# keonlee9420/Comprehensive-Transformer-TTS

Measured on AMD Instinct MI355X. Metric: mel-frames/sec (train step) LJSpeech batch=16, 1/2/4/8 MI355X, higher is better.
Workload: dtype f32; 1 GPU; LJSpeech transformer_fs2 batch=16/GPU seq<=128->mel<=1024x80; full train step fwd+loss+bwd+clip+Adam, dropout on; workload_detail=supervised durations (BASELINE configs[1]), global_batch=16, valid_frames_per_gpu=11992, padded_frames_per_gpu=16384, launch_mode=hipgraph(fwd+bwd | clip+adam), parallelism=dp1

## Files before the change

### comprehensive-transformer-tts_amd/_lib.py

```python
import ctypes as C
import os

_HERE = os.path.dirname(os.path.abspath(__file__))
LIB_PATH = os.environ.get("CTTS_LIB") or os.path.join(_HERE, "csrc", "libctts_hip.so")

_c_f32p = C.c_void_p
_i32, _i64, _f32, _u32, _vp = C.c_int32, C.c_int64, C.c_float, C.c_uint32, C.c_void_p


class GemmDesc(C.Structure):
    _fields_ = [
        ("A", _vp), ("B", _vp), ("C", _vp),
        ("M", _i32), ("N", _i32), ("K", _i32),
        ("lda", _i64), ("ldb", _i64), ("ldc", _i64),
        ("a_kc", _i32), ("b_kc", _i32),
        ("nb0", _i32), ("nb1", _i32),
        ("sA0", _i64), ("sA1", _i64), ("sB0", _i64), ("sB1", _i64), ("sC0", _i64), ("sC1", _i64),
        ("lens", _vp),
        ("lim_m", _i32), ("lim_n", _i32), ("lim_k", _i32),
        ("conv_T", _i32), ("conv_pad", _i32), ("conv_cin", _i32), ("conv_on_b", _i32),
        ("split_k", _i32),
        ("alpha", _f32),
        ("bias", _vp),
        ("Z", _vp), ("ldz", _i64),
# ... 56 lines not shown
    ]


class PsumTask(C.Structure):
    _fields_ = [("src", _vp), ("dst", _vp), ("n", _i64), ("stride", _i64), ("count", _i32), ("alpha", _f32)]


class SplitTask(C.Structure):
    _fields_ = [("src", _vp), ("dst", _vp), ("rows", _i64), ("cols", _i64), ("ld", _i64)]


class RepackTask(C.Structure):
    _fields_ = [("src", _vp), ("dst", _vp), ("cout", _i32), ("cin", _i32), ("k", _i32)]


_SIGNATURES = {
    "ctts_conv_dgrad_weights": [C.POINTER(RepackTask), C.c_int, _vp],
    "ctts_gemm_split_plan": [C.POINTER(GemmDesc), C.POINTER(_i32), C.POINTER(_i64)],
    "ctts_gemm_route": [C.POINTER(GemmDesc), C.POINTER(GemmRouteInfo)],
    "ctts_partial_sums": [C.POINTER(PsumTask), C.c_int, _vp],
    "ctts_reduce_parts": [C.c_int, _i64, C.c_int],
    "ctts_xcd_probe": [_vp, C.c_int, _vp],
    "ctts_posembed_fwd": [_vp, _vp, _vp, _vp, _vp, _vp, _i64, C.c_int, _f32, _vp, _u32, _vp],
    "ctts_posembed_bwd": [_vp, _vp, _vp, _vp, _vp, _vp, _i64, C.c_int, _f32, _vp, _u32, C.c_int, _vp, _vp],
    "ctts_gemm": [C.POINTER(GemmDesc), _vp],
    "ctts_gemm_takes_persistent": [C.POINTER(GemmDesc)],
    "ctts_gemm_ws_enable": [C.c_int],
    "ctts_gemm_takes_weight_stationary": [C.POINTER(GemmDesc)],
    "ctts_gemm_takes_bf16_split": [C.POINTER(GemmDesc)],
    "ctts_gemm_takes_planes": [C.POINTER(GemmDesc)],
    "ctts_split_planes": [C.POINTER(SplitTask), C.c_int, _vp],
# ... 111 lines not shown
    "ctts_comm_unique_id": [_vp],
    "ctts_comm_create": [C.POINTER(_vp), _i32, _i32, _vp],
    "ctts_comm_destroy": [_vp],
    "ctts_allreduce_mean": [_vp, _i64, _vp, _vp],
}
COMM_ID_BYTES = 128
EXPORTED_SYMBOLS = sorted(list(_SIGNATURES) + ["ctts_last_error", "ctts_version", "ctts_mha_supported", "ctts_relmha_workspace_floats",
                                               "ctts_mel_spectrogram_workspace_bytes", "ctts_gemm_workspace_bytes", "ctts_workspace_bytes",
                                               "ctts_workspace_error_word", "ctts_fastformer_workspace_floats",
                                               "ctts_griffinlim_workspace_bytes", "ctts_griffinlim_state_floats",
                                               "ctts_pitch_track_workspace_bytes", "ctts_trim_silence_workspace_bytes",
                                               "ctts_dtw_workspace_bytes", "ctts_loudness_workspace_bytes", "ctts_stoi_workspace_bytes",
                                               "ctts_si_sdr_workspace_bytes", "ctts_mr_stft_workspace_bytes",
                                               "ctts_batch_tile_map_ints", "ctts_conv2d_nhwc_workspace_bytes"])
ADAM_STATE_FLOATS = 3 + 2048
ABI_VERSION = 2

_lib = None


class CttsError(RuntimeError):
    pass


def load():
    global _lib
    if _lib is not None:
        return _lib
    if not os.path.exists(LIB_PATH):
        raise CttsError(
# ... 60 lines not shown
```

### comprehensive-transformer-tts_amd/csrc/optim.hip

```cpp
#include "ctts_common.h"

namespace {

__global__ __launch_bounds__(256) void sqnorm_kernel(const float4* __restrict__ g, long n4, const float* __restrict__ gtail, int ntail,
                                                      float* __restrict__ state) {
  float acc = 0.f;
  for (long i = (long)blockIdx.x * blockDim.x + threadIdx.x; i < n4; i += (long)gridDim.x * blockDim.x) {
    const float4 v = g[i];
    acc += v.x * v.x + v.y * v.y + v.z * v.z + v.w * v.w;
  }
  if (blockIdx.x == 0 && (int)threadIdx.x < ntail) acc += gtail[threadIdx.x] * gtail[threadIdx.x];
  acc = ctts_wave_sum(acc);
  __shared__ float s[4];
  if ((threadIdx.x & 63) == 0) s[threadIdx.x >> 6] = acc;
  __syncthreads();
  if (threadIdx.x == 0) state[3 + blockIdx.x] = (s[0] + s[1]) + (s[2] + s[3]);
}

__global__ __launch_bounds__(256) void sqnorm_reduce_kernel(float* __restrict__ state, int nparts) {
  __shared__ float s[256];
  float acc = 0.f;
  for (int i = threadIdx.x; i < nparts; i += 256) acc += state[3 + i];
  s[threadIdx.x] = acc;
  __syncthreads();
// ... 1 lines not shown
    if ((int)threadIdx.x < o) s[threadIdx.x] += s[threadIdx.x + o];
    __syncthreads();
  }
  if (threadIdx.x == 0) state[0] = s[0];
}

__device__ __forceinline__ void adam_one(float& p, float g, float& m, float& v, float coef, float wd, float b1, float b2, float eps,
                                         float step_size, float inv_sqrt_bc2) {
  g = g * coef + wd * p;
  m = b1 * m + (1.f - b1) * g;
  v = b2 * v + (1.f - b2) * g * g;
  const float denom = sqrtf(v) * inv_sqrt_bc2 + eps;
  p -= step_size * (m / denom);
}

__global__ __launch_bounds__(256) void adam_kernel(float* __restrict__ p, const float* __restrict__ g, float* __restrict__ m,
                                                    float* __restrict__ v, long n, const float* __restrict__ lr, float b1, float b2,
                                                    float eps, float wd, float max_norm, const float* __restrict__ state) {
  const float total = sqrtf(state[0]);
  float coef = 1.f;
  if (max_norm > 0.f) {
    const float c = max_norm / (total + 1e-6f);
    coef = c > 1.f ? 1.f : c;
  }
  const float step = state[1] + 1.f;
  const float bc1 = 1.f - powf(b1, step), bc2 = 1.f - powf(b2, step);
  const float step_size = lr[0] / bc1, inv_sqrt_bc2 = rsqrtf(bc2);
  const long n4 = n >> 2;
  float4* p4 = reinterpret_cast<float4*>(p);
  const float4* g4 = reinterpret_cast<const float4*>(g);
  float4* m4 = reinterpret_cast<float4*>(m);
  float4* v4 = reinterpret_cast<float4*>(v);
  for (long i = (long)blockIdx.x * blockDim.x + threadIdx.x; i < n4; i += (long)gridDim.x * blockDim.x) {
    float4 pp = p4[i], mm = m4[i], vv = v4[i];
    const float4 gg = g4[i];
    adam_one(pp.x, gg.x, mm.x, vv.x, coef, wd, b1, b2, eps, step_size, inv_sqrt_bc2);
    adam_one(pp.y, gg.y, mm.y, vv.y, coef, wd, b1, b2, eps, step_size, inv_sqrt_bc2);
    adam_one(pp.z, gg.z, mm.z, vv.z, coef, wd, b1, b2, eps, step_size, inv_sqrt_bc2);
    adam_one(pp.w, gg.w, mm.w, vv.w, coef, wd, b1, b2, eps, step_size, inv_sqrt_bc2);
    p4[i] = pp; m4[i] = mm; v4[i] = vv;
  }
  if (blockIdx.x == 0) {
    const long i = (n4 << 2) + threadIdx.x;
    if (i < n) adam_one(p[i], g[i], m[i], v[i], coef, wd, b1, b2, eps, step_size, inv_sqrt_bc2);
  }
}

__global__ void adam_finalize_kernel(float* __restrict__ state) {
  state[2] = sqrtf(state[0]);
  state[1] += 1.f;
}

}

extern "C" int ctts_adam_clip_step(float* p, const float* g, float* m, float* v, int64_t n, const float* lr, float beta1, float beta2,
                                   float eps, float weight_decay, float max_norm, float* state, void* stream) {
  CTTS_REQUIRE(p && g && m && v && lr && state && n >= 0, "ctts_adam_clip_step: bad arguments");
  auto al16 = [](const void* q) { return (reinterpret_cast<uintptr_t>(q) & 15) == 0; };
  CTTS_REQUIRE(al16(p) && al16(g) && al16(m) && al16(v), "ctts_adam_clip_step: arenas must be 16-byte aligned");
  if (n == 0) return 0;
  hipStream_t st = (hipStream_t)stream;
  const long n4 = n >> 2;
  const int blocks = (int)((n4 + 255) / 256 > CTTS_ADAM_PARTIALS ? CTTS_ADAM_PARTIALS : ((n4 + 255) / 256 < 1 ? 1 : (n4 + 255) / 256));
  hipLaunchKernelGGL(sqnorm_kernel, dim3(blocks), dim3(256), 0, st, (const float4*)g, n4, g + (n4 << 2), (int)(n - (n4 << 2)), state);
  CTTS_CHECK_LAUNCH("ctts_adam_clip_step(sqnorm)");
  hipLaunchKernelGGL(sqnorm_reduce_kernel, dim3(1), dim3(256), 0, st, state, blocks);
  CTTS_CHECK_LAUNCH("ctts_adam_clip_step(sqnorm reduce)");
  hipLaunchKernelGGL(adam_kernel, dim3(blocks), dim3(256), 0, st, p, g, m, v, (long)n, lr, beta1, beta2, eps, weight_decay, max_norm, state);
  CTTS_CHECK_LAUNCH("ctts_adam_clip_step(adam)");
  hipLaunchKernelGGL(adam_finalize_kernel, dim3(1), dim3(1), 0, st, state);
  CTTS_CHECK_LAUNCH("ctts_adam_clip_step(finalize)");
  return 0;
}

namespace {
__global__ __launch_bounds__(256) void mel_l1_fwd_kernel(const float* __restrict__ p1, const float* __restrict__ p2,
                                                          const float* __restrict__ tgt, const unsigned char* __restrict__ pad,
                                                          float* __restrict__ sums, float* __restrict__ roww, long rows, int C,
                                                          unsigned char* ws, int G) {
  const int lane = threadIdx.x & 63, wave = threadIdx.x >> 6;
  float a1 = 0.f, a2 = 0.f, aw = 0.f;
  for (long r = (long)blockIdx.x * 4 + wave; r < rows; r += (long)gridDim.x * 4) {
    const bool is_pad = pad[r] != 0;
    float s_t = 0.f, s1 = 0.f, s2 = 0.f;
    for (int c = lane; c < C; c += 64) {
      const float t = is_pad ? 0.f : tgt[r * C + c];
      const float x1 = is_pad ? 0.f : p1[r * C + c], x2 = is_pad ? 0.f : p2[r * C + c];
      s_t += fabsf(t); s1 += fabsf(x1 - t); s2 += fabsf(x2 - t);
    }
// ... 54 lines not shown
```

### comprehensive-transformer-tts_amd/dp.py

```python
import torch
import torch.distributed as dist


ARENA_ALIGN = 64


def arena_offsets(params):
    offs, o = [], 0
    for p in params:
        offs.append(o)
        o += (p.numel() + ARENA_ALIGN - 1) // ARENA_ALIGN * ARENA_ALIGN
    return offs, o


def _strided_like(flat_slice, p):
    if p.is_contiguous():
        return flat_slice.view_as(p)
    return flat_slice.as_strided(p.size(), p.stride())


class FlatGradArena:

    def __init__(self, params):
        items = list(params)
# ... 185 lines not shown
    def stop_timing(self):
        t, self._timing = self._timing, None
        if not t or not t["exposed"]:
            return None
        torch.cuda.synchronize()
        n = len(t["exposed"])
        per = [0.0] * len(self.ranges)
        for s, a, b in t["buckets"]:
            per[s] += a.elapsed_time(b)
        return {"allreduce_ms_per_bucket": [v / n for v in per], "bucket_bytes": self.bucket_bytes(),
                "exposed_ms_per_step": sum(a.elapsed_time(b) for a, b in t["exposed"]) / n, "steps": n,
                "note": "all-reduce time of a bucket is measured on the reducer's side stream (it overlaps the next backward stage); "
                        "exposed = stall of the compute stream at the join in front of the optimizer"}


class FlatAdam:

    def __init__(self, grad_arena, lr, betas=(0.9, 0.98), eps=1e-9, weight_decay=0.0, max_norm=1.0, current_step=0):
        from . import kernels
        self._k = kernels
        self.arena = grad_arena
        params = grad_arena.params
        dev = params[0].device
        n = grad_arena.flat.numel()
        self.flat_param = torch.zeros(n, dtype=torch.float32, device=dev)
        with torch.no_grad():
            for p, o in zip(params, grad_arena.offsets):
                v = _strided_like(self.flat_param[o:o + p.numel()], p)
                v.copy_(p.detach())
                p.data = v
        self.m = torch.zeros_like(self.flat_param)
        self.v = torch.zeros_like(self.flat_param)
        self.lr = lr if torch.is_tensor(lr) else torch.tensor(float(lr), dtype=torch.float32, device=dev)
        self.betas, self.eps, self.weight_decay, self.max_norm = betas, eps, weight_decay, max_norm
        from ._lib import ADAM_STATE_FLOATS
        self.state = torch.zeros(ADAM_STATE_FLOATS, dtype=torch.float32, device=dev)
        self.state[1] = float(current_step)

    def step(self):
        self._k.WEIGHTS_EPOCH[0] += 1
        self._k.adam_clip_step(self.flat_param, self.arena.flat, self.m, self.v, self.lr, self.betas[0], self.betas[1], self.eps,
                               self.weight_decay, self.max_norm, self.state)

    @property
    def total_norm(self):
        return self.state[2]

    def state_dict(self):
        step = float(self.state[1])
        st = {}
        for pos, p, o in zip(self.arena.positions, self.arena.params, self.arena.offsets):
            sl = slice(o, o + p.numel())
            st[pos] = {"step": torch.tensor(step), "exp_avg": _strided_like(self.m[sl], p).detach().clone(),
                       "exp_avg_sq": _strided_like(self.v[sl], p).detach().clone()}
        group = {"lr": float(self.lr), "betas": tuple(self.betas), "eps": self.eps, "weight_decay": self.weight_decay,
                 "amsgrad": False, "maximize": False, "foreach": None, "capturable": False, "differentiable": False, "fused": None,
                 "decoupled_weight_decay": False, "params": list(range(self.arena.n_all))}
# ... 37 lines not shown
```

### comprehensive-transformer-tts_amd/kernels.py

```python
import collections
import ctypes as C

import torch

from . import _lib
from ._lib import GemmDesc

ACT_NONE, ACT_RELU, ACT_GELU, ACT_TANH, ACT_SWISH = 0, 1, 2, 3, 4


def _stream():
    return C.c_void_p(torch.cuda.current_stream().cuda_stream)


def _p(t, offset=0):
    if t is None:
        return None
    if not t.is_cuda:
        raise _lib.CttsError("ctts kernels need device (HIP) tensors; got a CPU tensor - no CPU fallback exists")
    return t.data_ptr() + offset * t.element_size()


def _f32c(t, name):
    if t.dtype != torch.float32 or not t.is_contiguous():
# ... 413 lines not shown
                                       int(bool(write_all)), _p(tm), n, _stream()), "ctts_batch_tile_map")
    return tm


def conv_dgrad_weights(weights):
    if not weights:
        return []
    outs = [torch.empty(cin, k * cout, dtype=torch.float32, device=w.device) for w, cout, cin, k in weights]
    arr = (_lib.RepackTask * len(weights))()
    for t, (w, cout, cin, k), o in zip(arr, weights, outs):
        t.src, t.dst, t.cout, t.cin, t.k = _p(_f32c(w, "conv weight (GEMM-major)")), _p(o), int(cout), int(cin), int(k)
    _lib.check(_lib.load().ctts_conv_dgrad_weights(arr, len(arr), _stream()), "ctts_conv_dgrad_weights")
    return outs


def conv_weight_repack(src, dst, cout, cin, k, mode):
    lib = _lib.load()
    _lib.check(lib.ctts_conv_weight_repack(_p(src), _p(dst), cout, cin, k, mode, _stream()), "ctts_conv_weight_repack")
    return dst


def lr_index(dur, Tm, pad=None, round_mode=0, want_mel2ph=True):
    B, Ts = dur.shape
    is_float = dur.dtype == torch.float32
    if not is_float and dur.dtype != torch.int64:
        raise _lib.CttsError(f"lr_index: durations must be int64 or float32, got {dur.dtype}")
    dur = dur.contiguous()
    mel2ph = torch.empty(B, Tm, dtype=torch.int32, device=dur.device) if want_mel2ph else None
    mel_len = torch.empty(B, dtype=torch.int64, device=dur.device)
    cum = torch.empty(B, Ts, dtype=torch.int32, device=dur.device)
# ... 400 lines not shown
    _lib.check(lib.ctts_forward_sum_bwd(_p(attn_logprob), _p(in32), _p(out32), float(blank), _p(lse), _p(alpha), _p(nll),
                                        _p(_f32c(gscale, "gscale")), _p(grad), B, Tq, Tk, _stream()), "ctts_forward_sum_bwd")
    return grad


def adam_clip_step(p, g, m, v, lr, beta1, beta2, eps, weight_decay, max_norm, state):
    if state.numel() < _lib.ADAM_STATE_FLOATS or state.dtype != torch.float32:
        raise _lib.CttsError(f"adam_clip_step: state must hold CTTS_ADAM_STATE_FLOATS = {_lib.ADAM_STATE_FLOATS} float32 "
                             f"(got {state.numel()} {state.dtype}): the kernel writes its per-block norm partials behind the 3 scalars")
    if not (p.numel() == g.numel() == m.numel() == v.numel()):
        raise _lib.CttsError("adam_clip_step: p, g, m, v must have the same number of elements")
    lib = _lib.load()
    _lib.check(lib.ctts_adam_clip_step(_p(_f32c(p, "p")), _p(_f32c(g, "g")), _p(_f32c(m, "m")), _p(_f32c(v, "v")), p.numel(), _p(lr),
                                       float(beta1), float(beta2), float(eps), float(weight_decay), float(max_norm), _p(state),
                                       _stream()), "ctts_adam_clip_step")


def embedding_fwd(ids, weight):
    V, Cc = weight.shape
    ids = ids.contiguous()
    out = torch.empty(*ids.shape, Cc, dtype=torch.float32, device=weight.device)
    lib = _lib.load()
    _lib.check(lib.ctts_embedding_fwd(_p(ids), _p(_f32c(weight, "weight")), _p(out), ids.numel(), Cc, V, _stream()), "ctts_embedding_fwd")
    return out


def embedding_bwd(ids, dy, V, padding_idx=-1, acc_into=None):
    Cc = dy.shape[-1]
    dw = torch.empty(V, Cc, dtype=torch.float32, device=dy.device) if acc_into is None else acc_into
    lib = _lib.load()
# ... 1147 lines not shown
```

### comprehensive-transformer-tts_amd/ops.py

```python
import contextlib
import math
import os as _os

import torch

from . import kernels as K
from .kernels import ACT_NONE, ACT_RELU, ACT_GELU, ACT_TANH, ACT_SWISH


_FUSE_GRAD_ACCUM = False


def set_grad_accumulation_fusion(flag):
    global _FUSE_GRAD_ACCUM
    _FUSE_GRAD_ACCUM = bool(flag)


def grad_accumulation_fusion():
    return _FUSE_GRAD_ACCUM


def _grad_of(p):
    if not _FUSE_GRAD_ACCUM or p is None or not p.requires_grad:
        return None
# ... 203 lines not shown
               defer=fused and _WGRAD["stream"] is None, split_overwrite=not fused, **kw)
    return None if fused else dW


def _epilogue_bwd_stage(dY, Z, rowscale, seed, b, want_bias, has_res, delivered, act, alpha, p_drop, drop_offset):
    if delivered or (rowscale is None and act == ACT_NONE and p_drop == 0):
        dB = _param_colsum(dY.view(-1, dY.shape[-1]), b, alpha) if want_bias else None
        return dY, (dY if has_res else None), dB
    acc = _grad_of(b) if want_bias else None
    dZ, gm, dBn = K.epilogue_bwd(dY, rowscale, Z, act, p_drop, seed, drop_offset, want_gm=has_res and rowscale is not None,
                                 want_bias=want_bias, bias_scale=alpha, bias_acc_into=acc)
    d_res = (gm if rowscale is not None else dY) if has_res else None
    return dZ, d_res, (dBn if (want_bias and acc is None) else None)


def _conv_dgrad(dZ, w, x, dz_planes, pad, alpha, pr, rl):
    N, Cin, ksize = w.shape
    M, T, Kd = x.numel() // Cin, x.shape[-2], ksize * N
    pad_d = ksize - 1 - pad
    wd = _DGRAD_W.take(w, (Cin, Kd))
    if wd is None:
        wd = torch.empty(Cin, Kd, dtype=torch.float32, device=x.device)
        wmaj = _gemm_major(w)
        K.conv_weight_repack(wmaj if wmaj is not None else w.contiguous(), wd, N, Cin, ksize, 4 if wmaj is not None else 1)
    tiles = -(-M // 64) * -(-Cin // 64)
    sk = min(4, max(2, -(-2304 // tiles))) if (_DGRAD_SPLIT_K and tiles < 1536 and Kd >= 4096) else 1
    dX = torch.empty_like(x)
    args = (dZ, wd, dX, M, Cin, Kd, N, Kd, Cin, True, True)
    kw = dict(conv=(T, pad_d, N), alpha=alpha, row_halo=pad_d, split_k=1, split_overwrite=True, **rl)
    planes = _operand_planes("dgrad", w, args, kw, a_given=dz_planes)
    if planes:
        K.gemm(*args, **kw, **planes)
        return dX, planes["a_planes"]
    kw["tile_map"] = pr.tile_map(pad_d, M) if pr is not None else None
    if sk > 1 and not K.gemm_takes_persistent(*args, **kw):
        kw["split_k"] = sk
    K.gemm(*args, **kw)
    return dX, dz_planes


def _conv_wgrad(dZ, x, w, dz_planes, x_planes, pad, alpha, kmap, rl):
    N, Cin, ksize = w.shape
    M, T, Kd = x.numel() // Cin, x.shape[-2], ksize * Cin
    acc = _grad_of(w)
    fused = acc is not None
    gmaj = _gemm_major(acc) if fused else None
    dwf = gmaj if gmaj is not None else torch.empty(N, Kd, dtype=torch.float32, device=x.device)
    args = (dZ, x, dwf, N, Kd, M, N, Cin, Kd, False, False)
# ... 121 lines not shown

class _DgradCache(dict):

    def take(self, w, shape):
        ent = dict.pop(self, w.data_ptr(), None)
        if ent is None or ent[1] != _wstamp(w) or tuple(ent[0].shape) != tuple(shape):
            return None
        return ent[0]


_DGRAD_W = _DgradCache()

_PLANES = {"fwd": {}, "dgrad": {}, "want_fwd": set(), "want_dgrad": set()}


def _operand_planes(kind, w, args, kw, a_given=None):
    A, b_mat, _, M, N, Kdim, lda = args[:7]
    conv = kw.get("conv")
    if not K.plane_shape_ok(M, N, Kdim, conv[2] if conv is not None else None):
        return {}
    a_mat = A.view(M, lda)
    if not (a_mat.is_contiguous() and b_mat.is_contiguous() and lda % 32 == 0 and b_mat.shape[1] % 32 == 0):
        return {}
    if not K.gemm_takes_planes(*args, a_planes=_FakePlanes(a_mat), b_planes=_FakePlanes(b_mat), **kw):
        return {}
    ent = _PLANES[kind].get(w.data_ptr())
    if ent is not None and ent[1] == _wstamp(w) and ent[0].numel() == 3 * b_mat.numel():
        bp = ent[0]
    else:
        _PLANES["want_" + kind].add(w.data_ptr())
        bp = K.split_planes([b_mat])[0]
    return dict(a_planes=a_given if a_given is not None else K.split_planes([a_mat])[0], b_planes=bp)


def _wgrad_planes(args, kw, dz_pl, x_pl, cin):
    dZ, x, _, Mo, No, Kred = args[:6]
    if not K.plane_wgrad_shape_ok(Mo, No, Kred, cin) or not (dZ.is_contiguous() and x.is_contiguous()):
        return {}
    dz_mat, x_mat = dZ.view(Kred, Mo), x.view(Kred, cin)
    a = dz_pl if dz_pl is not None else _FakePlanes(dz_mat)
    b = x_pl if x_pl is not None else _FakePlanes(x_mat)
    if not K.gemm_takes_planes(*args, a_planes=a, b_planes=b, **kw):
        return {}
    made = iter(K.split_planes([m for m, pl in ((dz_mat, dz_pl), (x_mat, x_pl)) if pl is None]))
    return dict(a_planes=dz_pl if dz_pl is not None else next(made), b_planes=x_pl if x_pl is not None else next(made))
# ... 8 lines not shown
        return self._m.data_ptr()


def prepare_dgrad_weights(params):
    clear_dgrad_weights()
    params = list(params)
    live = {w.data_ptr() for w in params}
    _PLANES["want_fwd"] &= live
    _PLANES["want_dgrad"] &= live
    todo = []
    for w in params:
        wm = _gemm_major(w) if w.dim() == 3 else None
        if wm is not None and w.requires_grad:
            N, Cin, k = w.shape
            todo.append((w, (wm.detach(), N, Cin, k)))
    mats, slots = [], []
    for (w, (wm, _, _, _)), wd in zip(todo, K.conv_dgrad_weights([t for _, t in todo])):
        _DGRAD_W[w.data_ptr()] = (wd, _wstamp(w))
        if w.data_ptr() in _PLANES["want_fwd"]:
            mats.append(wm.contiguous()); slots.append(("fwd", w))
        if w.data_ptr() in _PLANES["want_dgrad"]:
            mats.append(wd); slots.append(("dgrad", w))
    for (kind, w), pl in zip(slots, K.split_planes(mats)):
        _PLANES[kind][w.data_ptr()] = (pl, _wstamp(w))


def clear_dgrad_weights():
    _DGRAD_W.clear()
    _PLANES["fwd"].clear()
    _PLANES["dgrad"].clear()


class PadRows:

    def __init__(self, lens, T):
        self.lens, self.T = lens, int(T)
        self._maps = {}
# ... 1087 lines not shown
```

### comprehensive-transformer-tts_amd/trainer.py

```python
import torch

from . import ops
from .dp import FlatGradArena, FlatAdam, BucketedReducer, stage_plan


class TrainStep:
    def __init__(self, model, loss_fn, optim, model_args, world=1, group=None, use_graph=True, overlap=True, n_cuts=3,
                 step_no=50001, fused_optimizer=True, max_norm=1.0, adam_step=0, force_staged=False, graph_collectives=None,
                 always_reduce=False, grad_acc_step=1):
        self.model, self.loss_fn, self.optim, self.world = model, loss_fn, optim, int(world)
        self.args = list(model_args)
        self.loss_inputs = [None, None] + list(self.args)
        self.step_no = step_no
        ops.set_grad_accumulation_fusion(True)
        self.arena = FlatGradArena(model.named_parameters())
        self.params = self.arena.params
        self.flat_grad = self.arena.flat
        self.use_graph = bool(use_graph)
        self.max_norm = max_norm
        self.grad_acc_step = max(1, int(grad_acc_step))
        self.g_opt_noclip = None
        import os as _os
        self._conv_weights = ([p for p in model.parameters() if p.dim() == 3 and p.requires_grad and ops._gemm_major(p) is not None]
                              if _os.environ.get("CTTS_BATCH_REPACK", "1") != "0" else [])
# ... 27 lines not shown
        args = list(self.args)
        if isinstance(args[7], dict):
            args[7] = dict(args[7])
        with ops.side_loss_scope():
            out = self.model(*args, step=self.step_no)
            inputs = list(self.loss_inputs)
            inputs[9:11] = out[-2:]
            losses = self.loss_fn(inputs, out[:-2], self.step_no)
        self.loss_val = losses[0].detach()
        self.loss_terms = losses
        return losses[0]

    def _stages(self):
        from . import kernels as _K
        try:
            if self._conv_weights:
                ops.prepare_dgrad_weights(self._conv_weights)
            rec = ops.CutRecorder(self.cut_names)
            with rec:
                loss = self._forward_loss()
            self.flat_grad.zero_()
            if self.grad_acc_step > 1:
                loss = loss * (1.0 / self.grad_acc_step)
            sink = _K.PartialSink()
            gen = rec.backward_stages(loss)
            while True:
                prev = _K.set_partial_sink(sink)
                try:
                    s = next(gen)
                    ops.join_side()
                    sink.flush()
# ... 51 lines not shown
                self._eager()
            self.ws_probe.poll_and_check()
            return
        graphs, gen, pool = [], self._stages(), None
        for s in range(self.n_stages):
            g = torch.cuda.CUDAGraph()
            with torch.cuda.graph(g, pool=pool, stream=side, capture_error_mode="thread_local"):
                got = next(gen)
            assert got == s
            pool = g.pool()
            graphs.append(g)
        for _ in gen:
            raise AssertionError("more backward stages than planned")
        self.graphs = graphs
        if self.fadam is not None:
            self.g_opt = torch.cuda.CUDAGraph()
            with torch.cuda.graph(self.g_opt, pool=pool, stream=side, capture_error_mode="thread_local"):
                self._optimizer_step(True)
            if self.grad_acc_step > 1:
                self.g_opt_noclip = torch.cuda.CUDAGraph()
                with torch.cuda.graph(self.g_opt_noclip, pool=pool, stream=side, capture_error_mode="thread_local"):
                    self._optimizer_step(False)
        self.ws_probe.poll_and_check()

    def bind_static_buffer(self, buf):
        self.static_buffer = buf

    def feed(self, device_buffer):
        self.static_buffer.copy_(device_buffer, non_blocking=True)

# ... 26 lines not shown
```

### include/ctts.h

```cpp
#ifndef CTTS_H
#define CTTS_H
#include <stddef.h>
#include <stdint.h>

#ifdef __cplusplus
extern "C" {
#endif

const char* ctts_last_error(void);
int ctts_version(void);

typedef struct ctts_gemm_desc {
  const float* A; const float* B; float* C;
  int32_t M, N, K;
  int64_t lda, ldb, ldc;
  int32_t a_kc, b_kc;
  int32_t nb0, nb1;
  int64_t sA0, sA1, sB0, sB1, sC0, sC1;
  const int32_t* lens;
  int32_t lim_m, lim_n, lim_k;
  int32_t conv_T, conv_pad, conv_cin, conv_on_b;
  int32_t split_k;
  float alpha;
  const float* bias;
// ... 182 lines not shown
                      const float* lambdas5, int cwt_l2, const int64_t* sil_ids3, const float* partials, const float* wsum,
                      const float* denoms, const float* g8, float* d_log_d, float* d_cwt, float* d_f0m, float* d_f0s, float* d_e,
                      void* stream);
int ctts_bin_loss_fwd(const float* soft, const float* hard, int64_t n, float* partials, float* out2, void* stream);
int ctts_bin_loss_bwd(const float* soft, const float* hard, const float* out2, const float* g, float* dsoft, int64_t n, void* stream);
int ctts_masked_loss_fwd(const float* pred, const float* target, const float* weight, int64_t n, int kind, float* partials, float* out2,
                         void* stream);
int ctts_masked_loss_bwd(const float* pred, const float* target, const float* weight, const float* out2, const float* g, float* dpred,
                         int64_t n, int kind, void* stream);

#define CTTS_ADAM_PARTIALS 2048
#define CTTS_ADAM_STATE_FLOATS (3 + CTTS_ADAM_PARTIALS)
int ctts_adam_clip_step(float* p, const float* g, float* m, float* v, int64_t n, const float* lr, float beta1, float beta2, float eps,
                        float weight_decay, float max_norm, float* state, void* stream);

int ctts_mel_l1_fwd(const float* p1, const float* p2, const float* tgt, const uint8_t* pad, float* sums, float* roww, int64_t rows,
                    int C, void* ws, void* stream);
int ctts_mel_l1_bwd(const float* p1, const float* p2, const float* tgt, const float* roww, const float* sums, const float* g, float* d1,
                    float* d2, int64_t rows, int C, void* stream);

typedef struct ctts_vconv_desc {
  const float* x;
  int64_t sxb, sxt, sxc;
  int32_t B, T, Cin, Cout, k, dil;
  int32_t transposed_u;
  int32_t act_in; float slope;
  const float* w; const uint16_t* w_planes;
  const float* bias;
  const float* R;
  float* out;
// ... 129 lines not shown
```

Baseline: 668,900 mel-frames/s.

## Fuse conv weight operand preparation into the Adam optimizer step

Adds an Adam kernel that, for conv weight segments, writes the updated weights directly into the forward bf16-split planes, the transposed dgrad weight matrix and its planes, while also folding the grad-norm reduction into the same kernel. This removes the separate per-step repack and plane-split passes that re-read all conv weights before the next forward/backward. It adds a segment table, a new operand cache keyed by weight pointer and stamp, and a stand-in matrix object, which brings extra complexity and the risk of stale operand caches.

```diff
diff --git a/comprehensive-transformer-tts_amd/_lib.py b/comprehensive-transformer-tts_amd/_lib.py
--- a/comprehensive-transformer-tts_amd/_lib.py
+++ b/comprehensive-transformer-tts_amd/_lib.py
@@ -94,7 +94,18 @@
     _fields_ = [("src", _vp), ("dst", _vp), ("cout", _i32), ("cin", _i32), ("k", _i32)]
 
 
+class WopTask(C.Structure):
+    _fields_ = [("src", _vp), ("fwd_planes", _vp), ("wd", _vp), ("wd_planes", _vp), ("cout", _i32), ("cin", _i32), ("k", _i32)]
+
+
+class AdamSeg(C.Structure):
+    _fields_ = [("offset", _i64), ("n", _i64), ("first_block", _i32), ("cout", _i32), ("cin", _i32), ("k", _i32),
+                ("fwd_planes", _vp), ("wd", _vp), ("wd_planes", _vp)]
+
+
 _SIGNATURES = {
+    "ctts_conv_weight_operands": [C.POINTER(WopTask), C.c_int, _vp],
+    "ctts_adam_clip_step_operands": [_vp, _vp, _vp, _vp, C.c_int64, _vp, _f32, _f32, _f32, _f32, _f32, _vp, _vp, C.c_int, C.c_int, _vp],
     "ctts_conv_dgrad_weights": [C.POINTER(RepackTask), C.c_int, _vp],
     "ctts_gemm_split_plan": [C.POINTER(GemmDesc), C.POINTER(_i32), C.POINTER(_i64)],
     "ctts_gemm_route": [C.POINTER(GemmDesc), C.POINTER(GemmRouteInfo)],
@@ -236,6 +247,9 @@
                                                "ctts_si_sdr_workspace_bytes", "ctts_mr_stft_workspace_bytes",
                                                "ctts_batch_tile_map_ints", "ctts_conv2d_nhwc_workspace_bytes"])
 ADAM_STATE_FLOATS = 3 + 2048
+WOP_CO, WOP_CI = 32, 256
+ADAM_STREAM_FLOATS = 4096
+ADAM_MAX_SEGS = 256
 ABI_VERSION = 2
 
 _lib = None
diff --git a/comprehensive-transformer-tts_amd/csrc/optim.hip b/comprehensive-transformer-tts_amd/csrc/optim.hip
--- a/comprehensive-transformer-tts_amd/csrc/optim.hip
+++ b/comprehensive-transformer-tts_amd/csrc/optim.hip
@@ -1,4 +1,5 @@
 #include "ctts_common.h"
+#include "planes_common.h"
 
 namespace {
 
@@ -39,18 +40,24 @@
   p -= step_size * (m / denom);
 }
 
-__global__ __launch_bounds__(256) void adam_kernel(float* __restrict__ p, const float* __restrict__ g, float* __restrict__ m,
-                                                    float* __restrict__ v, long n, const float* __restrict__ lr, float b1, float b2,
-                                                    float eps, float wd, float max_norm, const float* __restrict__ state) {
-  const float total = sqrtf(state[0]);
+struct AdamCoefs { float coef, step_size, inv_sqrt_bc2; };
+__device__ __forceinline__ AdamCoefs adam_coefs(float sumsq, float steps_done, float lr, float b1, float b2, float max_norm) {
+  const float total = sqrtf(sumsq);
   float coef = 1.f;
   if (max_norm > 0.f) {
     const float c = max_norm / (total + 1e-6f);
     coef = c > 1.f ? 1.f : c;
   }
-  const float step = state[1] + 1.f;
+  const float step = steps_done + 1.f;
   const float bc1 = 1.f - powf(b1, step), bc2 = 1.f - powf(b2, step);
-  const float step_size = lr[0] / bc1, inv_sqrt_bc2 = rsqrtf(bc2);
+  return {coef, lr / bc1, rsqrtf(bc2)};
+}
+
+__global__ __launch_bounds__(256) void adam_kernel(float* __restrict__ p, const float* __restrict__ g, float* __restrict__ m,
+                                                    float* __restrict__ v, long n, const float* __restrict__ lr, float b1, float b2,
+                                                    float eps, float wd, float max_norm, const float* __restrict__ state) {
+  const AdamCoefs c = adam_coefs(state[0], state[1], lr[0], b1, b2, max_norm);
+  const float coef = c.coef, step_size = c.step_size, inv_sqrt_bc2 = c.inv_sqrt_bc2;
   const long n4 = n >> 2;
   float4* p4 = reinterpret_cast<float4*>(p);
   const float4* g4 = reinterpret_cast<const float4*>(g);
@@ -76,6 +83,194 @@
   state[1] += 1.f;
 }
 
+constexpr int WOP_CO = CTTS_WOP_CO, WOP_CI = CTTS_WOP_CI;
+struct WopGeom {
+  int cout, cin, k;
+  uint16_t* fwd_planes;
+  float* wd;
+  uint16_t* wd_planes;
+};
+
+__device__ __forceinline__ int wop_col(int r, int c) { return c ^ (((r >> 3) & 3) << 4); }
+
+template <class Load8>
+__device__ __forceinline__ void wop_unit(const WopGeom& q, int unit, float* __restrict__ tile, Load8 load) {
+  const int tci = (q.cin + WOP_CI - 1) / WOP_CI;
+  const int cb = unit % tci;
+  unit /= tci;
+  const int kf = unit % q.k, co0 = (unit / q.k) * WOP_CO, ci0 = cb * WOP_CI;
+  const int cw = min(WOP_CI, q.cin - ci0);
+  const long ldf = (long)q.k * q.cin;
+  const int c = (threadIdx.x & 31) * 8;
+  if (c < cw) {
+    const int nv = min(8, cw - c);
+    for (int r = threadIdx.x >> 5; r < WOP_CO; r += 8) {
+      const int co = co0 + r;
+      if (co >= q.cout) break;
+      const long col = (long)kf * q.cin + ci0 + c;
+      float xs[8];
+      load(co * ldf + col, nv, xs);
+      if (q.fwd_planes) spl_store8(q.fwd_planes, co, ldf, col, xs);
+      float* t = tile + r * WOP_CI + wop_col(r, c);
+      *reinterpret_cast<float4*>(t) = make_float4(xs[0], xs[1], xs[2], xs[3]);
+      *reinterpret_cast<float4*>(t + 4) = make_float4(xs[4], xs[5], xs[6], xs[7]);
+    }
+  }
+  if (!q.wd && !q.wd_planes) return;
+  __syncthreads();
+  const int kk = q.k - 1 - kf;
+  const long ldd = (long)q.k * q.cout;
+  const bool vec = (q.cout & 7) == 0;
+  for (int item = threadIdx.x; item < cw * 4; item += 256) {
+    const int ci_l = item >> 2, g = item & 3, co = co0 + g * 8;
+    if (co >= q.cout) continue;
+    float xs[8];
+#pragma unroll
+    for (int j = 0; j < 8; ++j) xs[j] = tile[(g * 8 + j) * WOP_CI + wop_col(g * 8, ci_l)];
+    const long ci = ci0 + ci_l, col = (long)kk * q.cout + co;
+    if (vec) {
+      if (q.wd) {
+        float* o = q.wd + ci * ldd + col;
+        *reinterpret_cast<float4*>(o) = make_float4(xs[0], xs[1], xs[2], xs[3]);
+        *reinterpret_cast<float4*>(o + 4) = make_float4(xs[4], xs[5], xs[6], xs[7]);
+      }
+      if (q.wd_planes) spl_store8(q.wd_planes, ci, ldd, col, xs);
+    } else if (q.wd) {
+      for (int j = 0; j < 8 && co + j < q.cout; ++j) q.wd[ci * ldd + col + j] = xs[j];
+    }
+  }
+}
+
+constexpr int WOP_BATCH = 32;
+struct WopBatch {
+  const float* src[WOP_BATCH];
+  uint16_t* fwd_planes[WOP_BATCH];
+  float* wd[WOP_BATCH];
+  uint16_t* wd_planes[WOP_BATCH];
+  int cout[WOP_BATCH], cin[WOP_BATCH], k[WOP_BATCH];
+  int first_block[WOP_BATCH + 1];
+  int ntasks;
+};
+
+__global__ __launch_bounds__(256) void conv_weight_operands_kernel(const WopBatch b) {
+  __shared__ __attribute__((aligned(16))) float tile[WOP_CO * WOP_CI];
+  int t = 0;
+  while (t + 1 < b.ntasks && (int)blockIdx.x >= b.first_block[t + 1]) ++t;
+  const WopGeom q = {b.cout[t], b.cin[t], b.k[t], b.fwd_planes[t], b.wd[t], b.wd_planes[t]};
+  const float* __restrict__ src = b.src[t];
+  const bool vec = (q.cin & 3) == 0;
+  wop_unit(q, (int)blockIdx.x - b.first_block[t], tile, [&](long i, int nv, float (&xs)[8]) {
+    if (vec && nv == 8) {
+      const float4 x0 = *reinterpret_cast<const float4*>(src + i), x1 = *reinterpret_cast<const float4*>(src + i + 4);
+      xs[0] = x0.x; xs[1] = x0.y; xs[2] = x0.z; xs[3] = x0.w; xs[4] = x1.x; xs[5] = x1.y; xs[6] = x1.z; xs[7] = x1.w;
+    } else {
+#pragma unroll
+      for (int e = 0; e < 8; ++e) xs[e] = e < nv ? src[i + e] : 0.f;
+    }
+  });
+}
+
+__device__ __forceinline__ void adam_vec4(float4* p, const float4* g, float4* m, float4* v, long i, const AdamCoefs& c, float wd,
+                                          float b1, float b2, float eps, float4& pp) {
+  pp = p[i];
+  float4 mm = m[i], vv = v[i];
+  const float4 gg = g[i];
+  adam_one(pp.x, gg.x, mm.x, vv.x, c.coef, wd, b1, b2, eps, c.step_size, c.inv_sqrt_bc2);
+  adam_one(pp.y, gg.y, mm.y, vv.y, c.coef, wd, b1, b2, eps, c.step_size, c.inv_sqrt_bc2);
+  adam_one(pp.z, gg.z, mm.z, vv.z, c.coef, wd, b1, b2, eps, c.step_size, c.inv_sqrt_bc2);
+  adam_one(pp.w, gg.w, mm.w, vv.w, c.coef, wd, b1, b2, eps, c.step_size, c.inv_sqrt_bc2);
+  p[i] = pp; m[i] = mm; v[i] = vv;
+}
+
+__global__ __launch_bounds__(256) void adam_operands_kernel(float* __restrict__ p, const float* __restrict__ g, float* __restrict__ m,
+                                                             float* __restrict__ v, const float* __restrict__ lr, float b1, float b2,
+                                                             float eps, float wd, float max_norm, float* __restrict__ state, int nparts,
+                                                             const ctts_adam_seg* __restrict__ segs, int nsegs) {
+  __shared__ __attribute__((aligned(16))) float tile[WOP_CO * WOP_CI];
+  __shared__ int seg_of_block;
+  const int tid = threadIdx.x, blk = blockIdx.x;
+  if (tid < nsegs) {
+    const int lo = segs[tid].first_block, hi = tid + 1 < nsegs ? segs[tid + 1].first_block : (int)gridDim.x;
+    if (blk >= lo && blk < hi) seg_of_block = tid;
+  }
+  float acc = 0.f;
+  for (int i = tid; i < nparts; i += 256) acc += state[3 + i];
+  tile[tid] = acc;
+  __syncthreads();
+  for (int o = 128; o > 0; o >>= 1) {
+    if (tid < o) tile[tid] += tile[tid + o];
+    __syncthreads();
+  }
+  const float sumsq = tile[0];
+  const float steps_done = state[1];
+  const ctts_adam_seg q = segs[seg_of_block];
+  __syncthreads();
+  if (blk == 0 && tid == 0) state[0] = sumsq;
+  const AdamCoefs c = adam_coefs(sumsq, steps_done, lr[0], b1, b2, max_norm);
+  if (q.cout == 0) {
+    const long n4 = q.n >> 2;
+    float4* p4 = reinterpret_cast<float4*>(p + q.offset);
+    const float4* g4 = reinterpret_cast<const float4*>(g + q.offset);
+    float4* m4 = reinterpret_cast<float4*>(m + q.offset);
+    float4* v4 = reinterpret_cast<float4*>(v + q.offset);
+    const long i0 = (long)(blk - q.first_block) * (CTTS_ADAM_STREAM_FLOATS / 4);
+#pragma unroll
+    for (int u = 0; u < CTTS_ADAM_STREAM_FLOATS / 1024; ++u) {
+      const long i = i0 + u * 256 + tid;
+      float4 pp;
+      if (i < n4) adam_vec4(p4, g4, m4, v4, i, c, wd, b1, b2, eps, pp);
+    }
+    if (blk == q.first_block) {
+      const long i = q.offset + (n4 << 2) + tid;
+      if (i < q.offset + q.n) adam_one(p[i], g[i], m[i], v[i], c.coef, wd, b1, b2, eps, c.step_size, c.inv_sqrt_bc2);
+    }
+    return;
+  }
+  const WopGeom geo = {q.cout, q.cin, q.k, q.fwd_planes, q.wd, q.wd_planes};
+  float4* p4 = reinterpret_cast<float4*>(p + q.offset);
+  const float4* g4 = reinterpret_cast<const float4*>(g + q.offset);
+  float4* m4 = reinterpret_cast<float4*>(m + q.offset);
+  float4* v4 = reinterpret_cast<float4*>(v + q.offset);
+  wop_unit(geo, blk - q.first_block, tile, [&](long i, int, float (&xs)[8]) {
+    float4 x0, x1;
+    adam_vec4(p4, g4, m4, v4, i >> 2, c, wd, b1, b2, eps, x0);
+    adam_vec4(p4, g4, m4, v4, (i >> 2) + 1, c, wd, b1, b2, eps, x1);
+    xs[0] = x0.x; xs[1] = x0.y; xs[2] = x0.z; xs[3] = x0.w; xs[4] = x1.x; xs[5] = x1.y; xs[6] = x1.z; xs[7] = x1.w;
+  });
+}
+
+}
+
+extern "C" int ctts_conv_weight_operands(const ctts_wop_task* tasks, int ntasks, void* stream) {
+  CTTS_REQUIRE(ntasks >= 0 && (tasks || ntasks == 0), "ctts_conv_weight_operands: bad arguments");
+  auto al16 = [](const void* q) { return (reinterpret_cast<uintptr_t>(q) & 15) == 0; };
+  hipStream_t st = (hipStream_t)stream;
+  for (int t0 = 0; t0 < ntasks; t0 += WOP_BATCH) {
+    WopBatch b;
+    b.ntasks = 0;
+    long blocks = 0;
+    for (int t = t0; t < ntasks && t < t0 + WOP_BATCH; ++t) {
+      const ctts_wop_task& q = tasks[t];
+      CTTS_REQUIRE(q.src && q.cout > 0 && q.cin > 0 && q.k > 0 && al16(q.src) && al16(q.fwd_planes) && al16(q.wd) && al16(q.wd_planes),
+                   "ctts_conv_weight_operands: bad task %d (sizes > 0, 16-byte aligned pointers)", t);
+      CTTS_REQUIRE(!q.fwd_planes || ((long)q.k * q.cin % 32 == 0 && q.cin % 8 == 0),
+                   "ctts_conv_weight_operands: task %d: the plane set of wf needs k * cin %% 32 == 0 and cin %% 8 == 0", t);
+      CTTS_REQUIRE(!q.wd_planes || ((long)q.k * q.cout % 32 == 0 && q.cout % 8 == 0),
+                   "ctts_conv_weight_operands: task %d: the plane set of wd needs k * cout %% 32 == 0 and cout %% 8 == 0", t);
+      if (!q.fwd_planes && !q.wd && !q.wd_planes) continue;
+      const int i = b.ntasks++;
+      b.src[i] = q.src; b.fwd_planes[i] = q.fwd_planes; b.wd[i] = q.wd; b.wd_planes[i] = q.wd_planes;
+      b.cout[i] = q.cout; b.cin[i] = q.cin; b.k[i] = q.k;
+      b.first_block[i] = (int)blocks;
+      blocks += (long)CTTS_WOP_UNITS(q.cout, q.cin, q.k);
+      CTTS_REQUIRE(blocks < (1L << 30), "ctts_conv_weight_operands: too many elements in one call");
+    }
+    if (b.ntasks == 0) continue;
+    b.first_block[b.ntasks] = (int)blocks;
+    hipLaunchKernelGGL(conv_weight_operands_kernel, dim3((unsigned)blocks), dim3(256), 0, st, b);
+    CTTS_CHECK_LAUNCH("ctts_conv_weight_operands");
+  }
+  return 0;
 }
 
 extern "C" int ctts_adam_clip_step(float* p, const float* g, float* m, float* v, int64_t n, const float* lr, float beta1, float beta2,
@@ -98,6 +293,28 @@
   return 0;
 }
 
+extern "C" int ctts_adam_clip_step_operands(float* p, const float* g, float* m, float* v, int64_t n, const float* lr, float beta1,
+                                            float beta2, float eps, float weight_decay, float max_norm, float* state,
+                                            const ctts_adam_seg* segs, int nsegs, int nblocks, void* stream) {
+  CTTS_REQUIRE(p && g && m && v && lr && state && n >= 0, "ctts_adam_clip_step_operands: bad arguments");
+  auto al16 = [](const void* q) { return (reinterpret_cast<uintptr_t>(q) & 15) == 0; };
+  CTTS_REQUIRE(al16(p) && al16(g) && al16(m) && al16(v), "ctts_adam_clip_step_operands: arenas must be 16-byte aligned");
+  if (n == 0) return 0;
+  CTTS_REQUIRE(segs && nsegs > 0 && nsegs <= CTTS_ADAM_MAX_SEGS && nblocks > 0,
+               "ctts_adam_clip_step_operands: needs a table of 1 .. %d segments and its block count", CTTS_ADAM_MAX_SEGS);
+  hipStream_t st = (hipStream_t)stream;
+  const long n4 = n >> 2;
+  const int blocks = (int)((n4 + 255) / 256 > CTTS_ADAM_PARTIALS ? CTTS_ADAM_PARTIALS : ((n4 + 255) / 256 < 1 ? 1 : (n4 + 255) / 256));
+  hipLaunchKernelGGL(sqnorm_kernel, dim3(blocks), dim3(256), 0, st, (const float4*)g, n4, g + (n4 << 2), (int)(n - (n4 << 2)), state);
+  CTTS_CHECK_LAUNCH("ctts_adam_clip_step_operands(sqnorm)");
+  hipLaunchKernelGGL(adam_operands_kernel, dim3(nblocks), dim3(256), 0, st, p, g, m, v, lr, beta1, beta2, eps, weight_decay, max_norm,
+                     state, blocks, segs, nsegs);
+  CTTS_CHECK_LAUNCH("ctts_adam_clip_step_operands(adam)");
+  hipLaunchKernelGGL(adam_finalize_kernel, dim3(1), dim3(1), 0, st, state);
+  CTTS_CHECK_LAUNCH("ctts_adam_clip_step_operands(finalize)");
+  return 0;
+}
+
 namespace {
 __global__ __launch_bounds__(256) void mel_l1_fwd_kernel(const float* __restrict__ p1, const float* __restrict__ p2,
                                                           const float* __restrict__ tgt, const unsigned char* __restrict__ pad,
diff --git a/comprehensive-transformer-tts_amd/dp.py b/comprehensive-transformer-tts_amd/dp.py
--- a/comprehensive-transformer-tts_amd/dp.py
+++ b/comprehensive-transformer-tts_amd/dp.py
@@ -223,9 +223,28 @@
                         "exposed = stall of the compute stream at the join in front of the optimizer"}
 
 
+def conv_segments(params, offsets):
+    out = []
+    for p, o in zip(params, offsets):
+        if p.dim() == 3:
+            cout, cin, k = p.shape
+            if (p.stride() == (k * cin, 1, cin) or (k == 1 and p.is_contiguous())) and cin % 8 == 0:
+                out.append((p, o, cout, cin, k))
+    return out
+
+
+def operand_wants(convs, base_ptr, want_fwd, want_dgrad):
+    from .kernels import wop_planes_ok
+    out = []
+    for _, off, cout, cin, k in convs:
+        ptr = base_ptr + 4 * off
+        out.append((ptr in want_fwd and wop_planes_ok(cout, k, cin), ptr in want_dgrad and wop_planes_ok(cin, k, cout)))
+    return tuple(out)
+
+
 class FlatAdam:
 
-    def __init__(self, grad_arena, lr, betas=(0.9, 0.98), eps=1e-9, weight_decay=0.0, max_norm=1.0, current_step=0):
+    def __init__(self, grad_arena, lr, betas=(0.9, 0.98), eps=1e-9, weight_decay=0.0, max_norm=1.0, current_step=0, emit_operands=None):
         from . import kernels
         self._k = kernels
         self.arena = grad_arena
@@ -245,11 +264,67 @@
         from ._lib import ADAM_STATE_FLOATS
         self.state = torch.zeros(ADAM_STATE_FLOATS, dtype=torch.float32, device=dev)
         self.state[1] = float(current_step)
+        import os
+        env = os.environ.get("CTTS_ADAM_OPERANDS")
+        self._convs = conv_segments(params, grad_arena.offsets) if (emit_operands is not False and env != "0") else []
+        if emit_operands is None and env is None and 2 * sum(c * ci * k for _, _, c, ci, k in self._convs) < n:
+            self._convs = []
+        self.emit_operands = bool(self._convs)
+        self._op_key, self._op_bufs, self._op_table = None, [], None
+        kernels.WEIGHTS_EPOCH[0] += 1
+        if self._convs:
+            import weakref
+            from . import ops
+            weakref.finalize(self, ops._OPT_OPERANDS.drop, [p.data_ptr() for p, *_ in self._convs])
 
     def step(self):
         self._k.WEIGHTS_EPOCH[0] += 1
-        self._k.adam_clip_step(self.flat_param, self.arena.flat, self.m, self.v, self.lr, self.betas[0], self.betas[1], self.eps,
-                               self.weight_decay, self.max_norm, self.state)
+        if not self._convs:
+            self._k.adam_clip_step(self.flat_param, self.arena.flat, self.m, self.v, self.lr, self.betas[0], self.betas[1], self.eps,
+                                   self.weight_decay, self.max_norm, self.state)
+            return
+        self.size_operands()
+        table, nsegs, nblocks = self._op_table
+        self._k.adam_clip_step_operands(self.flat_param, self.arena.flat, self.m, self.v, self.lr, self.betas[0], self.betas[1],
+                                        self.eps, self.weight_decay, self.max_norm, self.state, table, nsegs, nblocks)
+        self._register_operands()
+
+    def size_operands(self):
+        if not self._convs:
+            return
+        from . import ops
+        key = operand_wants(self._convs, self.flat_param.data_ptr(), ops._PLANES["want_fwd"], ops._PLANES["want_dgrad"])
+        if key == self._op_key:
+            return
+        if self.flat_param.is_cuda and torch.cuda.is_current_stream_capturing():
+            raise RuntimeError("FlatAdam.step: the set of conv weights whose GEMMs run on the plane kernel changed since the operand "
+                               "buffers were sized; run one eager step (or FlatAdam.refresh_operands()) before capturing the optimizer")
+        dev, k = self.flat_param.device, self._k
+        bufs = []
+        for (_, off, cout, cin, ks), (wf, wdp) in zip(self._convs, key):
+            bufs.append((k.new_planes(cout, ks * cin, dev) if wf else None,
+                         None if wdp else torch.empty(cin, ks * cout, dtype=torch.float32, device=dev),
+                         k.new_planes(cin, ks * cout, dev) if wdp else None))
+        rows, nblocks = k.adam_segment_table(self.flat_param.numel(), [
+            (off, cout, cin, ks) + tuple(0 if b is None else b.data_ptr() for b in bs) for (_, off, cout, cin, ks), bs in zip(self._convs, bufs)])
+        self._op_key, self._op_bufs, self._op_table = key, bufs, (k.adam_segments_to_device(rows, dev), len(rows), nblocks)
+
+    def _register_operands(self):
+        from . import ops
+        for (p, _, _, _, _), (fwd, wd, dgrad) in zip(self._convs, self._op_bufs):
+            ops._OPT_OPERANDS.register(p, fwd, wd, dgrad)
+
+    def operands_current(self, weights):
+        from . import ops
+        return bool(self._convs) and all(ops._OPT_OPERANDS.valid(w) for w in weights)
+
+    def refresh_operands(self):
+        if not self._convs:
+            return
+        from . import ops
+        self.size_operands()
+        self._k.conv_weight_operands([(ops._gemm_major(p).detach(), c, ci, ks) for p, _, c, ci, ks in self._convs], out=self._op_bufs)
+        self._register_operands()
 
     @property
     def total_norm(self):
diff --git a/comprehensive-transformer-tts_amd/kernels.py b/comprehensive-transformer-tts_amd/kernels.py
--- a/comprehensive-transformer-tts_amd/kernels.py
+++ b/comprehensive-transformer-tts_amd/kernels.py
@@ -451,6 +451,31 @@
     return outs
 
 
+def wop_planes_ok(rows, k, cols):
+    return (k * cols) % 32 == 0 and cols % 8 == 0
+
+
+def conv_weight_operands(weights, fwd_planes=True, wd=True, wd_planes=True, out=None):
+    if not weights:
+        return []
+    n = len(weights)
+    if out is None:
+        per = [f if isinstance(f, (list, tuple)) else [f] * n for f in (fwd_planes, wd, wd_planes)]
+        out = []
+        for (w, cout, cin, k), wf, wwd, wp in zip(weights, *per):
+            out.append((new_planes(cout, k * cin, w.device) if wf else None,
+                        torch.empty(cin, k * cout, dtype=torch.float32, device=w.device) if wwd else None,
+                        new_planes(cin, k * cout, w.device) if wp else None))
+    arr = (_lib.WopTask * n)()
+    for t, (w, cout, cin, k), (fp, d, dp) in zip(arr, weights, out):
+        if (fp is not None and not wop_planes_ok(cout, k, cin)) or (dp is not None and not wop_planes_ok(cin, k, cout)):
+            raise _lib.CttsError(f"conv_weight_operands: no plane set for the weight ({cout}, {cin}, {k})")
+        t.src, t.cout, t.cin, t.k = _p(_f32c(w, "conv weight (GEMM-major)")), int(cout), int(cin), int(k)
+        t.fwd_planes, t.wd, t.wd_planes = (None if x is None else x.data_ptr() for x in (fp, d, dp))
+    _lib.check(_lib.load().ctts_conv_weight_operands(arr, n, _stream()), "ctts_conv_weight_operands")
+    return out
+
+
 def conv_weight_repack(src, dst, cout, cin, k, mode):
     lib = _lib.load()
     _lib.check(lib.ctts_conv_weight_repack(_p(src), _p(dst), cout, cin, k, mode, _stream()), "ctts_conv_weight_repack")
@@ -881,6 +906,58 @@
     _lib.check(lib.ctts_adam_clip_step(_p(_f32c(p, "p")), _p(_f32c(g, "g")), _p(_f32c(m, "m")), _p(_f32c(v, "v")), p.numel(), _p(lr),
                                        float(beta1), float(beta2), float(eps), float(weight_decay), float(max_norm), _p(state),
                                        _stream()), "ctts_adam_clip_step")
+
+
+def wop_units(cout, cin, k):
+    return -(-cout // _lib.WOP_CO) * k * -(-cin // _lib.WOP_CI)
+
+
+def adam_segment_table(n, convs):
+    rows, blocks, pos = [], 0, 0
+
+    def plain(a, b):
+        nonlocal blocks
+        if b > a:
+            rows.append((a, b - a, blocks, 0, 0, 0, 0, 0, 0))
+            blocks += max(1, -(-((b - a) // 4) // (_lib.ADAM_STREAM_FLOATS // 4)))
+
+    for off, cout, cin, k, fp, d, dp in sorted(convs):
+        ne = cout * cin * k
+        if off < pos or off + ne > n or off % 4 or cin % 8 or min(cout, cin, k) <= 0:
+            raise _lib.CttsError(f"adam_segment_table: conv segment at {off} ({cout}, {cin}, {k}) overlaps, leaves the arena of {n} floats, "
+                                 "is not 16-byte aligned or has cin % 8 != 0")
+        if (fp and not wop_planes_ok(cout, k, cin)) or (dp and not wop_planes_ok(cin, k, cout)):
+            raise _lib.CttsError(f"adam_segment_table: no plane set for the weight ({cout}, {cin}, {k})")
+        plain(pos, off)
+        rows.append((off, ne, blocks, cout, cin, k, fp, d, dp))
+        blocks += wop_units(cout, cin, k)
+        pos = off + ne
+    plain(pos, n)
+    if len(rows) > _lib.ADAM_MAX_SEGS:
+        raise _lib.CttsError(f"adam_segment_table: {len(rows)} segments, the kernel takes {_lib.ADAM_MAX_SEGS}")
+    return rows, blocks
+
+
+def adam_segments_to_device(rows, device):
+    arr = (_lib.AdamSeg * len(rows))()
+    for t, r in zip(arr, rows):
+        t.offset, t.n, t.first_block, t.cout, t.cin, t.k = r[:6]
+        t.fwd_planes, t.wd, t.wd_planes = (x or None for x in r[6:])
+    return torch.frombuffer(bytearray(bytes(arr)), dtype=torch.uint8).to(device)
+
+
+def adam_clip_step_operands(p, g, m, v, lr, beta1, beta2, eps, weight_decay, max_norm, state, seg_table, nsegs, nblocks):
+    if state.numel() < _lib.ADAM_STATE_FLOATS or state.dtype != torch.float32:
+        raise _lib.CttsError(f"adam_clip_step_operands: state must hold CTTS_ADAM_STATE_FLOATS = {_lib.ADAM_STATE_FLOATS} float32")
+    if not (p.numel() == g.numel() == m.numel() == v.numel()):
+        raise _lib.CttsError("adam_clip_step_operands: p, g, m, v must have the same number of elements")
+    if seg_table.numel() != nsegs * C.sizeof(_lib.AdamSeg) or seg_table.device != p.device:
+        raise _lib.CttsError("adam_clip_step_operands: the segment table does not hold `nsegs` entries on the parameters' device")
+    lib = _lib.load()
+    _lib.check(lib.ctts_adam_clip_step_operands(_p(_f32c(p, "p")), _p(_f32c(g, "g")), _p(_f32c(m, "m")), _p(_f32c(v, "v")), p.numel(),
+                                                _p(lr), float(beta1), float(beta2), float(eps), float(weight_decay), float(max_norm),
+                                                _p(state), _p(seg_table), int(nsegs), int(nblocks), _stream()),
+               "ctts_adam_clip_step_operands")
 
 
 def embedding_fwd(ids, weight):
diff --git a/comprehensive-transformer-tts_amd/ops.py b/comprehensive-transformer-tts_amd/ops.py
--- a/comprehensive-transformer-tts_amd/ops.py
+++ b/comprehensive-transformer-tts_amd/ops.py
@@ -1,6 +1,7 @@
 import contextlib
 import math
 import os as _os
+import weakref
 
 import torch
 
@@ -241,15 +242,24 @@
     return dZ, d_res, (dBn if (want_bias and acc is None) else None)
 
 
+def _repack_dgrad_weight(w, device):
+    N, Cin, ksize = w.shape
+    wd = torch.empty(Cin, ksize * N, dtype=torch.float32, device=device)
+    wmaj = _gemm_major(w)
+    K.conv_weight_repack(wmaj if wmaj is not None else w.contiguous(), wd, N, Cin, ksize, 4 if wmaj is not None else 1)
+    return wd
+
+
 def _conv_dgrad(dZ, w, x, dz_planes, pad, alpha, pr, rl):
     N, Cin, ksize = w.shape
     M, T, Kd = x.numel() // Cin, x.shape[-2], ksize * N
     pad_d = ksize - 1 - pad
     wd = _DGRAD_W.take(w, (Cin, Kd))
     if wd is None:
-        wd = torch.empty(Cin, Kd, dtype=torch.float32, device=x.device)
-        wmaj = _gemm_major(w)
-        K.conv_weight_repack(wmaj if wmaj is not None else w.contiguous(), wd, N, Cin, ksize, 4 if wmaj is not None else 1)
+        wd = _OPT_OPERANDS.get(w, "wd")
+    if wd is None:
+        pl = _OPT_OPERANDS.get(w, "dgrad")
+        wd = _MatrixStandIn(pl, Cin, Kd) if pl is not None else _repack_dgrad_weight(w, x.device)
     tiles = -(-M // 64) * -(-Cin // 64)
     sk = min(4, max(2, -(-2304 // tiles))) if (_DGRAD_SPLIT_K and tiles < 1536 and Kd >= 4096) else 1
     dX = torch.empty_like(x)
@@ -259,6 +269,8 @@
     if planes:
         K.gemm(*args, **kw, **planes)
         return dX, planes["a_planes"]
+    if isinstance(wd, _MatrixStandIn):
+        args = (dZ, _repack_dgrad_weight(w, x.device)) + args[2:]
     kw["tile_map"] = pr.tile_map(pad_d, M) if pr is not None else None
     if sk > 1 and not K.gemm_takes_persistent(*args, **kw):
         kw["split_k"] = sk
@@ -410,6 +422,45 @@
 _PLANES = {"fwd": {}, "dgrad": {}, "want_fwd": set(), "want_dgrad": set()}
 
 
+class _OptOperands(dict):
+
+    def register(self, w, fwd, wd, dgrad):
+        self[w.data_ptr()] = (_wstamp(w), tuple(w.shape), {"fwd": fwd, "wd": wd, "dgrad": dgrad}, weakref.ref(w))
+
+    def valid(self, w):
+        ent = dict.get(self, w.data_ptr())
+        return ent is not None and ent[3]() is w and ent[0] == _wstamp(w) and ent[1] == tuple(w.shape)
+
+    def drop(self, ptrs):
+        for ptr in ptrs:
+            dict.pop(self, ptr, None)
+
+    def get(self, w, kind):
+        return dict.get(self, w.data_ptr())[2][kind] if self.valid(w) else None
+
+
+_OPT_OPERANDS = _OptOperands()
+
+
+class _MatrixStandIn:
+    is_cuda = True
+
+    def __init__(self, planes, rows, cols):
+        self._pl, self.shape, self.device = planes, (rows, cols), planes.device
+
+    def data_ptr(self):
+        return self._pl.data_ptr()
+
+    def element_size(self):
+        return 4
+
+    def numel(self):
+        return self.shape[0] * self.shape[1]
+
+    def is_contiguous(self):
+        return True
+
+
 def _operand_planes(kind, w, args, kw, a_given=None):
     A, b_mat, _, M, N, Kdim, lda = args[:7]
     conv = kw.get("conv")
@@ -420,11 +471,16 @@
         return {}
     if not K.gemm_takes_planes(*args, a_planes=_FakePlanes(a_mat), b_planes=_FakePlanes(b_mat), **kw):
         return {}
-    ent = _PLANES[kind].get(w.data_ptr())
-    if ent is not None and ent[1] == _wstamp(w) and ent[0].numel() == 3 * b_mat.numel():
+    bp = _OPT_OPERANDS.get(w, kind)
+    ent = _PLANES[kind].get(w.data_ptr()) if bp is None else None
+    if bp is not None and bp.numel() == 3 * b_mat.numel():
+        pass
+    elif ent is not None and ent[1] == _wstamp(w) and ent[0].numel() == 3 * b_mat.numel():
         bp = ent[0]
     else:
         _PLANES["want_" + kind].add(w.data_ptr())
+        if isinstance(b_mat, _MatrixStandIn):
+            return {}
         bp = K.split_planes([b_mat])[0]
     return dict(a_planes=a_given if a_given is not None else K.split_planes([a_mat])[0], b_planes=bp)
 
@@ -463,13 +519,19 @@
         if wm is not None and w.requires_grad:
             N, Cin, k = w.shape
             todo.append((w, (wm.detach(), N, Cin, k)))
+    want_f = [w.data_ptr() in _PLANES["want_fwd"] for w, _ in todo]
+    want_d = [w.data_ptr() in _PLANES["want_dgrad"] for w, _ in todo]
+    fused_f = [f and K.wop_planes_ok(N, k, Cin) for f, (_, (_, N, Cin, k)) in zip(want_f, todo)]
+    fused_d = [d and K.wop_planes_ok(Cin, k, N) for d, (_, (_, N, Cin, k)) in zip(want_d, todo)]
+    made = K.conv_weight_operands([t for _, t in todo], fwd_planes=fused_f, wd=True, wd_planes=fused_d)
     mats, slots = [], []
-    for (w, (wm, _, _, _)), wd in zip(todo, K.conv_dgrad_weights([t for _, t in todo])):
+    for (w, (wm, _, _, _)), (fp, wd, dp), wf, wdg in zip(todo, made, want_f, want_d):
         _DGRAD_W[w.data_ptr()] = (wd, _wstamp(w))
-        if w.data_ptr() in _PLANES["want_fwd"]:
-            mats.append(wm.contiguous()); slots.append(("fwd", w))
-        if w.data_ptr() in _PLANES["want_dgrad"]:
-            mats.append(wd); slots.append(("dgrad", w))
+        for kind, pl, want, mat in (("fwd", fp, wf, wm), ("dgrad", dp, wdg, wd)):
+            if pl is not None:
+                _PLANES[kind][w.data_ptr()] = (pl, _wstamp(w))
+            elif want:
+                mats.append(mat.contiguous()); slots.append((kind, w))
     for (kind, w), pl in zip(slots, K.split_planes(mats)):
         _PLANES[kind][w.data_ptr()] = (pl, _wstamp(w))
 
diff --git a/comprehensive-transformer-tts_amd/trainer.py b/comprehensive-transformer-tts_amd/trainer.py
--- a/comprehensive-transformer-tts_amd/trainer.py
+++ b/comprehensive-transformer-tts_amd/trainer.py
@@ -65,7 +65,7 @@
     def _stages(self):
         from . import kernels as _K
         try:
-            if self._conv_weights:
+            if self._conv_weights and not (self.fadam is not None and self.fadam.operands_current(self._conv_weights)):
                 ops.prepare_dgrad_weights(self._conv_weights)
             rec = ops.CutRecorder(self.cut_names)
             with rec:
@@ -147,6 +147,7 @@
             raise AssertionError("more backward stages than planned")
         self.graphs = graphs
         if self.fadam is not None:
+            self.fadam.size_operands()
             self.g_opt = torch.cuda.CUDAGraph()
             with torch.cuda.graph(self.g_opt, pool=pool, stream=side, capture_error_mode="thread_local"):
                 self._optimizer_step(True)
diff --git a/include/ctts.h b/include/ctts.h
--- a/include/ctts.h
+++ b/include/ctts.h
@@ -220,6 +220,23 @@
 int ctts_adam_clip_step(float* p, const float* g, float* m, float* v, int64_t n, const float* lr, float beta1, float beta2, float eps,
                         float weight_decay, float max_norm, float* state, void* stream);
 
+#define CTTS_WOP_CO 32
+#define CTTS_WOP_CI 256
+#define CTTS_WOP_UNITS(cout, cin, k) ((((cout) + CTTS_WOP_CO - 1) / CTTS_WOP_CO) * (k) * (((cin) + CTTS_WOP_CI - 1) / CTTS_WOP_CI))
+typedef struct ctts_wop_task { const float* src; uint16_t* fwd_planes; float* wd; uint16_t* wd_planes; int32_t cout, cin, k; } ctts_wop_task;
+int ctts_conv_weight_operands(const ctts_wop_task* tasks, int ntasks, void* stream);
+
+#define CTTS_ADAM_STREAM_FLOATS 4096
+#define CTTS_ADAM_MAX_SEGS 256
+typedef struct ctts_adam_seg {
+  int64_t offset, n;
+  int32_t first_block, cout, cin, k;
+  uint16_t* fwd_planes; float* wd; uint16_t* wd_planes;
+} ctts_adam_seg;
+int ctts_adam_clip_step_operands(float* p, const float* g, float* m, float* v, int64_t n, const float* lr, float beta1, float beta2,
+                                 float eps, float weight_decay, float max_norm, float* state, const ctts_adam_seg* segs, int nsegs,
+                                 int nblocks, void* stream);
+
 int ctts_mel_l1_fwd(const float* p1, const float* p2, const float* tgt, const uint8_t* pad, float* sums, float* roww, int64_t rows,
                     int C, void* ws, void* stream);
 int ctts_mel_l1_bwd(const float* p1, const float* p2, const float* tgt, const float* roww, const float* sums, const float* g, float* d1,
```

New measurement: 672,800 mel-frames/s (median of 6 runs). About the same (+0.6%).
